# izhengfan/se2lam

Measured on NVIDIA H100. Metric: ORB keypoints/sec at 640x480 (8-level pyramid, 1000 kps/frame), higher is better.
Workload: dtype u8

## Files before the change

### se2lam_b200/csrc/orb.cu

```cuda
#include <cuda.h>

#include <algorithm>
#include <cmath>
#include <cstring>
#include <type_traits>
#include <vector>

#include "blur_px.h"
#include "common.h"
#include "fast_screen.h"
#include "introselect.h"
#include "resp_key.h"

namespace {

using se2gpu::fail;

constexpr int EDGE = 16;
constexpr int HALF_PATCH = 15;
constexpr int PATCH = 31;
constexpr int MAX_LEVELS = 16;
constexpr int FAST_THREADS = 256;
constexpr int ORB_LANES = 4;
constexpr int BLUR_WARPS = 4;
constexpr int BLUR_TH = 48;

__device__ const signed char d_pattern[1024] = {
#include "orb_pattern_31.inc"
};
__constant__ int c_umax[16];
__constant__ int c_vmax[16];
__constant__ float c_gauss[7];

struct LevelGeo {
    int w, h, pitch;
    size_t plane_off;
    int nDesired, cols, rows, nCells, nfeaturesCell;
    int cell_base;
    int kp_off, kp_cap;
    float scale, kp_size;
    int tab_off;
    int tile_base;
    int blur_th, blur_strips;
    int fbw, fbh;
    int sel_off, sel_cap;
};

struct CellGeo {
    int level, x0, y0, x1, y1;
    int skipped;
    int cand_off, cand_cap;
};

struct TileGeo { int level, strip, cg; };

struct CellHdr { int n_base, n_a, n_b, pad; };

struct OrbDev {
    int nlevels, nfeatures, fast_th, t_lo;
    int n_cells, n_tiles;
    const LevelGeo* levels;
    const CellGeo* cells;
    const TileGeo* tiles;
    const int* itab;
    const short* stab;
    uint8_t* plain;
    uint8_t* blurred;
    size_t frame_plane_bytes;
    uint32_t* cand;
    size_t cand_total;
    CellHdr* hdr;
    uint32_t* lkp;
    int lkp_total;
    int* lcount;
    uint64_t* sel;
    int sel_total;
    int* err;
    int frame0;
};

__device__ __forceinline__ int reflect101(int p, int len) {
    if (len == 1) return 0;
    while (p < 0 || p >= len) p = p < 0 ? -p : 2 * (len - 1) - p;
    return p;
}

constexpr int PYR0_ROWS = 4;
__global__ void __launch_bounds__(256) orb_pyr0(OrbDev d, LevelGeo L, const uint8_t* __restrict__ imgs, int stride, size_t frame_stride, int nvec) {
    const int tid = threadIdx.y * 64 + threadIdx.x;
    const int f = blockIdx.z + d.frame0;
    const uint8_t* img = imgs + f * frame_stride;
    uint8_t* plane = d.plain + f * d.frame_plane_bytes + L.plane_off;
    const int rows = L.h + 2 * EDGE;
    if (blockIdx.x + 1 < gridDim.x) {
        const int vx = blockIdx.x * 64 + threadIdx.x;
        const int y0 = (blockIdx.y * 4 + threadIdx.y) * PYR0_ROWS;
        if (vx >= nvec) return;
        uint4 v[PYR0_ROWS];
#pragma unroll
        for (int k = 0; k < PYR0_ROWS; ++k)
            if (y0 + k < rows) v[k] = __ldg(reinterpret_cast<const uint4*>(img + (size_t)reflect101(y0 + k - EDGE, L.h) * stride) + vx);
#pragma unroll
        for (int k = 0; k < PYR0_ROWS; ++k)
            if (y0 + k < rows) *reinterpret_cast<uint4*>(plane + (size_t)(y0 + k) * L.pitch + EDGE + 16 * vx) = v[k];
        return;
    }
    const int tail0 = EDGE + 16 * nvec, nw = 4 + (L.pitch - tail0) / 4;
    for (int item = tid; item < 4 * PYR0_ROWS * nw; item += 256) {
// ... 590 lines not shown
            if (nToRetain[k] & SEL_NOMORE) continue;
            const int t = nTotal[k];
            if (t > nNew) nToRetain[k] = nNew;
            else { nToRetain[k] = t | SEL_NOMORE; dist += nNew - t; ++more; }
        }
        nToDistribute = warp_sum(dist); nNoMore += warp_sum(more);
    }
    int before = 0, all = 0;
    for (int k = lane; k < nCells; k += 32) {
        const int kept = min(nTotal[k], nToRetain[k] & ~SEL_NOMORE);
        all += kept;
        if (k < me) before += kept;
    }
    before = warp_sum(before); all = warp_sum(all);
    __syncwarp();
    const int cap = L.sel_cap;
    if (me == 0 && lane == 0) {
        if (all > cap) *d.err = 2;
        d.lcount[f * d.nlevels + level] = min(all, cap);
    }
    const int tot = nTotal[me], n = nToRetain[me] & ~SEL_NOMORE, kept = min(tot, n);
    if (kept <= 0 || before >= cap) return;
    R* g;
    if constexpr (HARRIS) g = hb.cand64 + (size_t)f * d.cand_total + c.cand_off;
    else g = d.cand + (size_t)f * d.cand_total + c.cand_off;
    R* v = g;
    if (tot > n) {
        if (tot <= stage_n) {
            v = stage;
            for (int i = lane; i < tot; i += 32) v[i] = g[i];
            __syncwarp();
        }
        se2gpu::kp_nth_element_warp<K>(v, tot, n - 1, wq[wid]);
    }
    R* out = reinterpret_cast<R*>(d.sel) + (size_t)f * d.sel_total + L.sel_off + before;
    for (int i = lane; i < kept && before + i < cap; i += 32) out[i] = v[i];
}

template <bool HARRIS>
__global__ void __launch_bounds__(32) orb_select_levels(OrbDev d, HarrisBufs hb) {
    typedef typename std::conditional<HARRIS, se2gpu::KpKey64, se2gpu::KpScore32>::type K;
    typedef typename K::rec R;
    extern __shared__ __align__(16) uint8_t sell_smem[];
    __shared__ int wq[128];
    asm volatile("griddepcontrol.launch_dependents;" ::: "memory");
    const int lane = threadIdx.x, level = blockIdx.x, f = blockIdx.y + d.frame0;
    const LevelGeo& L = d.levels[level];
    R* v = reinterpret_cast<R*>(sell_smem);
    const R* g = reinterpret_cast<const R*>(d.sel) + (size_t)f * d.sel_total + L.sel_off;
    int* lc = d.lcount + f * d.nlevels + level;
    asm volatile("griddepcontrol.wait;" ::: "memory");
    int total = *lc;
    for (int i = lane; i < total; i += 32) v[i] = g[i];
    __syncwarp();
    if (total > L.nDesired) {
        se2gpu::kp_nth_element_warp<K>(v, total, L.nDesired - 1, wq);
        total = L.nDesired;
    }
    uint32_t* out = d.lkp + (size_t)f * d.lkp_total + L.kp_off;
    if constexpr (HARRIS) {
        float* resp = hb.lresp + (size_t)f * d.lkp_total + L.kp_off;
        for (int i = lane; i < total; i += 32) { const R r = v[i]; out[i] = (uint32_t)r; resp[i] = se2gpu::resp_from_key((uint32_t)(r >> 32)); }
    } else {
        for (int i = lane; i < total; i += 32) out[i] = v[i];
    }
    __syncwarp();
    if (lane == 0) *lc = total;
}

__global__ void __launch_bounds__(128) orb_debug_nth(uint32_t* v, const int* __restrict__ offs, const int* __restrict__ nth, int count) {
    __shared__ int wq[4][128];
    const int k = blockIdx.x * 4 + (threadIdx.x >> 5);
    if (k >= count) return;
    se2gpu::kp_nth_element_warp(v + offs[k], offs[k + 1] - offs[k], nth[k], wq[threadIdx.x >> 5]);
}

__global__ void __launch_bounds__(128) orb_debug_nth64(uint64_t* v, const int* __restrict__ offs, const int* __restrict__ nth, int count) {
    __shared__ int wq[4][128];
    const int k = blockIdx.x * 4 + (threadIdx.x >> 5);
    if (k >= count) return;
    se2gpu::kp_nth_element_warp<se2gpu::KpKey64>(v + offs[k], offs[k + 1] - offs[k], nth[k], wq[threadIdx.x >> 5]);
}

__global__ void __launch_bounds__(BLUR_WARPS * 32, 4) orb_blur(OrbDev d, int tile0, int tile_end) {
    const int tile = tile0 + blockIdx.x * BLUR_WARPS + (threadIdx.x >> 5);
    if (tile >= tile_end) return;
    const TileGeo t = d.tiles[tile];
    const LevelGeo& L = d.levels[t.level];
    const int pitch = L.pitch, Lw = L.w, Lh = L.h, th = L.blur_th, strips = L.blur_strips, ncg = pitch / 8;
    int s = t.strip, cg = t.cg + (threadIdx.x & 31);
    while (cg >= ncg) { cg -= ncg; ++s; }
    if (s >= strips) return;
    const int x8 = 8 * cg;
    const size_t off = (size_t)(blockIdx.y + d.frame0) * d.frame_plane_bytes + L.plane_off + x8;
    const uint8_t* __restrict__ src = d.plain + off;
    uint8_t* __restrict__ dst = d.blurred + off;
    if (s == 0)
        for (int y = 0; y < EDGE; ++y) *reinterpret_cast<uint2*>(dst + (size_t)y * pitch) = __ldg(reinterpret_cast<const uint2*>(src + (size_t)y * pitch));
    if (s == strips - 1)
        for (int y = EDGE + Lh; y < Lh + 2 * EDGE; ++y) *reinterpret_cast<uint2*>(dst + (size_t)y * pitch) = __ldg(reinterpret_cast<const uint2*>(src + (size_t)y * pitch));
    uint32_t m0 = 0, m1 = 0;
#pragma unroll
    for (int q = 0; q < 4; ++q) {
        m0 |= (x8 + q >= EDGE && x8 + q < EDGE + Lw) ? (0xFFu << (8 * q)) : 0u;
        m1 |= (x8 + 4 + q >= EDGE && x8 + 4 + q < EDGE + Lw) ? (0xFFu << (8 * q)) : 0u;
    }
    const int y0 = EDGE + min(s * th, Lh - th);
    const uint8_t* rp = src + (size_t)(y0 - 3) * pitch;
    uint8_t* wp = dst + (size_t)y0 * pitch;
    float hr[7][8];
    uint2 cw[7];
    uint2 nc = __ldg(reinterpret_cast<const uint2*>(rp));
    uint32_t nl = __ldg(reinterpret_cast<const uint32_t*>(rp - 4)), nr = __ldg(reinterpret_cast<const uint32_t*>(rp + 8));
    auto row = [&](const int k) {
        const uint2 c = nc;
        const uint32_t l = nl, r = nr;
        rp += pitch;
        nc = __ldg(reinterpret_cast<const uint2*>(rp));
        nl = __ldg(reinterpret_cast<const uint32_t*>(rp - 4));
        nr = __ldg(reinterpret_cast<const uint32_t*>(rp + 8));
        float b[14];
#pragma unroll
        for (int j = 0; j < 3; ++j) b[j] = blurpx::byte_to_float(l, j + 1);
#pragma unroll
        for (int j = 0; j < 4; ++j) { b[3 + j] = blurpx::byte_to_float(c.x, j); b[7 + j] = blurpx::byte_to_float(c.y, j); }
#pragma unroll
        for (int j = 0; j < 3; ++j) b[11 + j] = blurpx::byte_to_float(r, j);
#pragma unroll
        for (int q = 0; q < 8; ++q) {
            float a = __fmul_rn(c_gauss[0], b[q]);
            a = __fmaf_rn(c_gauss[1], b[q + 1], a); a = __fmaf_rn(c_gauss[2], b[q + 2], a); a = __fmaf_rn(c_gauss[3], b[q + 3], a);
            a = __fmaf_rn(c_gauss[4], b[q + 4], a); a = __fmaf_rn(c_gauss[5], b[q + 5], a); a = __fmaf_rn(c_gauss[6], b[q + 6], a);
            hr[k][q] = a;
        }
        cw[k] = c;
    };
    auto out = [&](const int k) {
        unsigned o[8];
#pragma unroll
        for (int q = 0; q < 8; ++q) {
            float a = __fmul_rn(c_gauss[3], hr[(k + 4) % 7][q]);
            a = __fmaf_rn(c_gauss[4], __fadd_rn(hr[(k + 5) % 7][q], hr[(k + 3) % 7][q]), a);
            a = __fmaf_rn(c_gauss[5], __fadd_rn(hr[(k + 6) % 7][q], hr[(k + 2) % 7][q]), a);
            a = __fmaf_rn(c_gauss[6], __fadd_rn(hr[k][q], hr[(k + 1) % 7][q]), a);
            o[q] = blurpx::round_sat_bits(a);
        }
        const uint2 ctr = cw[(k + 4) % 7];
        const uint32_t v0 = blurpx::pack_low_bytes(o[0], o[1], o[2], o[3]), v1 = blurpx::pack_low_bytes(o[4], o[5], o[6], o[7]);
        *reinterpret_cast<uint2*>(wp) = make_uint2((v0 & m0) | (ctr.x & ~m0), (v1 & m1) | (ctr.y & ~m1));
        wp += pitch;
    };
#pragma unroll
    for (int k = 0; k < 7; ++k) row(k);
    out(6);
    for (int i = 1; i < th; i += 7) {
#pragma unroll
        for (int k = 0; k < 7; ++k) { row(k); out(k); }
    }
}

__device__ __forceinline__ float fast_atan2_deg(float y, float x) {
    const float p1 = 0.9997878412794807f * (float)(180 / M_PI);
    const float p3 = -0.3258083974640975f * (float)(180 / M_PI);
    const float p5 = 0.1555786518463281f * (float)(180 / M_PI);
    const float p7 = -0.04432655554792128f * (float)(180 / M_PI);
    const float ax = fabsf(x), ay = fabsf(y);
    float a, c, c2;
    if (ax >= ay) {
        c = __fdiv_rn(ay, __fadd_rn(ax, (float)2.2204460492503131e-16));
        c2 = __fmul_rn(c, c);
        a = __fmul_rn(__fadd_rn(__fmul_rn(__fadd_rn(__fmul_rn(__fadd_rn(__fmul_rn(p7, c2), p5), c2), p3), c2), p1), c);
    } else {
        c = __fdiv_rn(ax, __fadd_rn(ay, (float)2.2204460492503131e-16));
        c2 = __fmul_rn(c, c);
        a = __fsub_rn(90.f, __fmul_rn(__fadd_rn(__fmul_rn(__fadd_rn(__fmul_rn(__fadd_rn(__fmul_rn(p7, c2), p5), c2), p3), c2), p1), c));
    }
    if (x < 0) a = __fsub_rn(180.f, a);
    if (y < 0) a = __fsub_rn(360.f, a);
    return a;
}

template <bool HARRIS>
__global__ void __launch_bounds__(256) orb_orient_describe(OrbDev d, se2gpu_keypoint* __restrict__ kps, uint8_t* __restrict__ desc,
                                                           int* __restrict__ counts, const float* __restrict__ lresp) {
    __shared__ float4 patf[256];
    for (int i = threadIdx.x; i < 256; i += blockDim.x) patf[(i & 7) * 32 + (i >> 3)] = make_float4((float)d_pattern[4 * i], (float)d_pattern[4 * i + 1], (float)d_pattern[4 * i + 2], (float)d_pattern[4 * i + 3]);
    __syncthreads();
    asm volatile("griddepcontrol.wait;" ::: "memory");
    const int f = blockIdx.y + d.frame0;
    const int slot = blockIdx.x * (blockDim.x >> 5) + (threadIdx.x >> 5);
    const int lane = threadIdx.x & 31;
    const int* lc = d.lcount + f * d.nlevels;
    int level = -1, off = 0, total = 0;
    for (int l = 0; l < d.nlevels; ++l) {
        const int c = lc[l];
        if (level < 0 && slot < total + c) { level = l; off = total; }
        total += c;
    }
    if (slot == 0 && lane == 0) counts[f] = total;
    if (level < 0) return;
    const LevelGeo& L = d.levels[level];
    const size_t kslot = (size_t)f * d.lkp_total + L.kp_off + (slot - off);
    const uint32_t rec = d.lkp[kslot];
    const int x = rec & 0xFFF, y = (rec >> 12) & 0xFFF, score = rec >> 24;
    const size_t base = f * d.frame_plane_bytes + L.plane_off + (size_t)(EDGE + y) * L.pitch + (EDGE + x);
    const uint8_t* center = d.plain + base;
    int m10 = 0, m01 = 0;
    if (lane < 31) {
        const int u = lane - HALF_PATCH, vm = c_vmax[abs(u)];
        const uint8_t* col = center + u;
        const int pitch = L.pitch;
        int colsum = col[0];
#pragma unroll
        for (int v0 = 1; v0 <= HALF_PATCH; v0 += 5) {
            int p[5], m[5];
#pragma unroll
            for (int k = 0; k < 5; ++k) {
                const int off = min(v0 + k, vm) * pitch;
                p[k] = col[off]; m[k] = col[-off];
            }
#pragma unroll
            for (int k = 0; k < 5; ++k)
                if (v0 + k <= vm) { colsum += p[k] + m[k]; m01 += (v0 + k) * (p[k] - m[k]); }
        }
        m10 = u * colsum;
    }
#pragma unroll
    for (int o = 16; o > 0; o >>= 1) { m10 += __shfl_xor_sync(0xffffffffu, m10, o); m01 += __shfl_xor_sync(0xffffffffu, m01, o); }
    const float angle = fast_atan2_deg((float)m01, (float)m10);
    const float factorPI = (float)(M_PI / 180.f);
    const float ang = __fmul_rn(angle, factorPI);
    double sd, cd;
    sincos((double)ang, &sd, &cd);
    const float a = (float)cd, b = (float)sd;
    const uint8_t* bc = d.blurred + base;
    unsigned val = 0;
    int o0[8], o1[8];
#pragma unroll
    for (int k = 0; k < 8; ++k) {
        const float4 pt = patf[k * 32 + lane];
        const float x0 = pt.x, y0 = pt.y, x1 = pt.z, y1 = pt.w;
        const int r0 = __float2int_rn(__fadd_rn(__fmul_rn(x0, b), __fmul_rn(y0, a)));
        const int c0 = __float2int_rn(__fsub_rn(__fmul_rn(x0, a), __fmul_rn(y0, b)));
        const int r1 = __float2int_rn(__fadd_rn(__fmul_rn(x1, b), __fmul_rn(y1, a)));
        const int c1 = __float2int_rn(__fsub_rn(__fmul_rn(x1, a), __fmul_rn(y1, b)));
        o0[k] = r0 * L.pitch + c0; o1[k] = r1 * L.pitch + c1;
    }
    int t0[8], t1[8];
#pragma unroll
    for (int k = 0; k < 8; ++k) { t0[k] = bc[o0[k]]; t1[k] = bc[o1[k]]; }
#pragma unroll
    for (int k = 0; k < 8; ++k) val |= (unsigned)(t0[k] < t1[k]) << k;
    unsigned w = val;
    w |= __shfl_down_sync(0xffffffffu, val, 1) << 8;
    w |= __shfl_down_sync(0xffffffffu, val, 2) << 16;
    w |= __shfl_down_sync(0xffffffffu, val, 3) << 24;
    const size_t oslot = (size_t)f * d.nfeatures + slot;
    if ((lane & 3) == 0) reinterpret_cast<unsigned*>(desc + oslot * 32)[lane >> 2] = w;
    if (lane == 0) {
        se2gpu_keypoint kp;
        kp.x = level ? __fmul_rn((float)x, L.scale) : (float)x;
        kp.y = level ? __fmul_rn((float)y, L.scale) : (float)y;
        kp.size = L.kp_size; kp.angle = angle; kp.response = HARRIS ? lresp[kslot] : (float)score; kp.octave = level; kp.class_id = -1;
        kps[oslot] = kp;
    }
}

inline int cv_round_f(float v) { return (int)lrintf(v); }

}

struct se2gpu_orb {
    int device = 0, nfeatures = 0, nlevels = 0, fast_th = 20, max_w = 0, max_h = 0, max_batch = 0;
    bool harris = false;
    double scaleFactor = 1.2;
    std::vector<float> mvScaleFactor, mvInvScaleFactor;
    std::vector<int> mnFeaturesPerLevel;
    int cur_w = -1, cur_h = -1;
    std::vector<LevelGeo> levels;
    std::vector<CellGeo> cells;
    std::vector<TileGeo> tiles;
    size_t fast_smem = 0, select_smem = 0, select_levels_smem = 0, resize_w_smem = 0;
    int sel_max_cells = 0;
    int sel_stage_n = 0;
    int resize_rows = 0, resize_raw_pitch = 0;
    int resize_tall_rows = 0; size_t resize_tall_smem = 0;
    int resize_tall_ctas = 0;
    bool fast_big = false;
    bool fast_tma = false;
    size_t fast_tma_smem = 0;
    FastMaps fast_maps{};
    bool und_on = false;
    float und_K[9] = {}, und_D[14] = {};
    int und_nd = 0, und_w = 0, und_h = 0;
    short2* d_und_m1 = nullptr; uint16_t* d_und_m2 = nullptr; size_t und_cap = 0;
    size_t cap_plane = 0, cap_cand = 0, cap_cells = 0, cap_tiles = 0, cap_tab = 0, cap_lkp = 0, cap_sel = 0;
    OrbDev d{};
    LevelGeo* d_levels = nullptr; CellGeo* d_cells = nullptr; TileGeo* d_tiles = nullptr; int* d_itab = nullptr; short* d_stab = nullptr;

    uint8_t* d_in = nullptr; se2gpu_keypoint* d_kps = nullptr; uint8_t* d_desc = nullptr; int* d_counts = nullptr;
    HarrisBufs hb{};
    se2gpu::DeviceBuffers bufs;
    int last_n = 0;
    se2gpu::Profiler prof;
    cudaStream_t side = nullptr;
    cudaEvent_t ev_pyr = nullptr, ev_blur = nullptr;
    cudaStream_t pipe[ORB_LANES] = {};
    int* pin_counts = nullptr; se2gpu_keypoint* pin_kps = nullptr; uint8_t* pin_desc = nullptr;
    struct Pending { bool on = false; int n = 0, lanes = 0; bool pipelined = false; se2gpu_keypoint* kps = nullptr; uint8_t* desc = nullptr; int* counts = nullptr;
                     se2gpu_keypoint* out_kps = nullptr; uint8_t* out_desc = nullptr; int* out_counts = nullptr; } pend;
    se2gpu_orb* twin = nullptr;
    int submit_next = 0, wait_next = 0, in_flight = 0;
    int create_args[9] = {};
};

namespace {

int build_geometry(se2gpu_orb* h, int w, int hgt, bool dry, size_t* plane_bytes, size_t* cand_total, size_t* n_cells,
                   size_t* n_tiles, size_t* tab_total, size_t* max_fast_smem,
                   std::vector<LevelGeo>* Lv, std::vector<CellGeo>* Cv, std::vector<TileGeo>* Tv, bool* fast_big_out = nullptr,
                   size_t* fast_tma_smem_out = nullptr) {
    (void)dry;
    const int nl = h->nlevels;
    std::vector<LevelGeo> L(nl);
    std::vector<CellGeo> C;
    std::vector<TileGeo> T;
    size_t poff = 0, coff = 0, toff = 0, fsm = 0, fsm_big = 0, fsm_tma = 0;
    bool fast_big = false;
    bool tma_ok = true;
    int kp_off = 0, sel_off = 0;
    const float imageRatio = (float)w / (float)hgt;
    for (int l = 0; l < nl; ++l) {
        LevelGeo& g = L[l];
        const float scale = h->mvInvScaleFactor[l];
        g.w = cv_round_f((float)w * scale); g.h = cv_round_f((float)hgt * scale);
        if (g.w < 2 * EDGE + 7 || g.h < 2 * EDGE + 7) return fail(SE2GPU_ERR_INVALID, "level %d of a %dx%d frame is %dx%d: too small for the 16 px border", l, w, hgt, g.w, g.h);
        if (g.w + 2 * EDGE > 4095 || g.h + 2 * EDGE > 4095) return fail(SE2GPU_ERR_CAPACITY, "frames wider/taller than 4063 px are not supported");
        g.pitch = (g.w + 2 * EDGE + 31) & ~31;
        g.plane_off = poff;
        poff += (size_t)g.pitch * (g.h + 2 * EDGE);
        poff = (poff + 255) & ~(size_t)255;
        g.nDesired = h->mnFeaturesPerLevel[l];
        g.cols = (int)sqrtf((float)g.nDesired / (5 * imageRatio));
        g.rows = (int)(imageRatio * g.cols);
        if (g.cols < 1 || g.rows < 1) return fail(SE2GPU_ERR_INVALID, "level %d has a %dx%d cell grid (nfeatures too small): undefined in the reference", l, g.cols, g.rows);
        const int minB = EDGE, maxBX = g.w - EDGE, maxBY = g.h - EDGE;
        const int W = maxBX - minB, H = maxBY - minB;
        const int cellW = (int)ceilf((float)W / g.cols), cellH = (int)ceilf((float)H / g.rows);
        g.nCells = g.rows * g.cols;
        g.nfeaturesCell = (int)ceilf((float)g.nDesired / g.nCells);
        g.cell_base = (int)C.size();
        g.kp_off = kp_off; g.kp_cap = g.nDesired; kp_off += g.nDesired;
        g.scale = h->mvScaleFactor[l];
        g.kp_size = (float)(int)(PATCH * h->mvScaleFactor[l]);
        g.tab_off = (int)toff; toff += (size_t)g.w + g.h;
        std::vector<int> iniXCol(g.cols, 0);
        const size_t first_cell = C.size();
        int max_cw = 0, max_ch = 0;
        float hY = cellH + 6;
        for (int i = 0; i < g.rows; ++i) {
            const float iniY = minB + i * cellH - 3;
            bool rowSkipped = false;
            if (i == g.rows - 1) { hY = maxBY + 3 - iniY; if (hY <= 0) rowSkipped = true; }
            float hX = cellW + 6;
            for (int j = 0; j < g.cols; ++j) {
                CellGeo c{};
                c.level = l;
                if (rowSkipped) { c.skipped = 1; C.push_back(c); continue; }
                float iniX;
                if (i == 0) { iniX = minB + j * cellW - 3; iniXCol[j] = (int)iniX; } else iniX = iniXCol[j];
                if (j == g.cols - 1) { hX = maxBX + 3 - iniX; if (hX <= 0) { c.skipped = 1; C.push_back(c); continue; } }
                const int r0 = (int)iniY, r1 = (int)(iniY + hY), c0 = (int)iniX, c1 = (int)(iniX + hX);
                if (r1 > g.h || c1 > g.w || r0 < 0 || c0 < 0) return fail(SE2GPU_ERR_INVALID, "cell grid of level %d leaves the image (the reference asserts here)", l);
                c.x0 = c0 + 3; c.x1 = c1 - 3; c.y0 = r0 + 3; c.y1 = r1 - 3;
                const int cw = std::max(c.x1 - c.x0, 0), chh = std::max(c.y1 - c.y0, 0);
                c.cand_off = (int)coff;
                c.cand_cap = ((cw + 1) / 2) * ((chh + 1) / 2) + 8;
                coff += c.cand_cap;
                if (cw > 0 && chh > 0) {
                    max_cw = std::max(max_cw, ((c.x0 - 3 + EDGE) & 15) + cw); max_ch = std::max(max_ch, chh);
                    const size_t pwb = (size_t)((cw + 6 + 3 + 3) / 4 + 1) * 4;
                    const size_t bitmap = (size_t)chh * fastpx::nms_words_per_row(cw) * 4;
                    if (pwb * (chh + 6) > 65535) fast_big = true;
                    fsm = std::max(fsm, ((pwb * (chh + 6) + 15) & ~(size_t)15) + (((size_t)fastpx::nms_plane_bytes((int)pwb, chh) + 15) & ~(size_t)15) + bitmap + (size_t)cw * chh * 2 + 64);
                    const size_t nchunk = (size_t)chh * ((cw + 31) / 32);
                    fsm_big = std::max(fsm_big, ((pwb * (chh + 6) + 15) & ~(size_t)15) + (((size_t)(cw + 2) * (chh + 2) + 15) & ~(size_t)15) + nchunk * 4 + 64);
                }
                C.push_back(c);
            }
        }
        g.fbw = (max_cw + 6 + 15) & ~15; g.fbh = max_ch + 6;
        if (max_cw > 0) {
            if (g.fbw > 256 || g.fbh > 256 || (size_t)g.fbw * g.fbh > 65535) tma_ok = false;
            for (size_t ci = first_cell; ci < C.size(); ++ci) {
                const int cw = C[ci].x1 - C[ci].x0, chh = C[ci].y1 - C[ci].y0;
                if (C[ci].skipped || cw <= 0 || chh <= 0) continue;
                const size_t pw = (size_t)g.fbw, bitmap = (size_t)chh * fastpx::nms_words_per_row(cw) * 4;
                fsm_tma = std::max(fsm_tma, (size_t)128 + ((pw * g.fbh + 15) & ~(size_t)15) + (((size_t)fastpx::nms_plane_bytes(g.fbw, chh) + 15) & ~(size_t)15) + bitmap + (size_t)cw * chh * 2 + 64);
            }
        }
        g.sel_cap = 2 * g.nDesired + 4 * g.nCells + 64;
        g.sel_off = sel_off; sel_off += g.sel_cap;
        g.tile_base = (int)T.size();
        g.blur_strips = std::max(2, (g.h + BLUR_TH - 1) / BLUR_TH);
        g.blur_th = ((g.h + g.blur_strips - 1) / g.blur_strips + 12) / 7 * 7 - 6;
        for (int it = 0; it < g.blur_strips * (g.pitch / 8); it += 32) T.push_back(TileGeo{l, it / (g.pitch / 8), it % (g.pitch / 8)});
    }
    *plane_bytes = poff; *cand_total = coff; *n_cells = C.size(); *n_tiles = T.size(); *tab_total = toff;
    if (fsm > 227 * 1024) fast_big = true;
    *max_fast_smem = fast_big ? fsm_big : fsm;
    if (fast_big_out) *fast_big_out = fast_big;
    if (fast_tma_smem_out) *fast_tma_smem_out = (tma_ok && !fast_big && fsm_tma <= 227 * 1024) ? fsm_tma : 0;
    if (Lv) *Lv = L;
    if (Cv) *Cv = C;
    if (Tv) *Tv = T;
    return SE2GPU_OK;
}

typedef CUresult (*EncodeTiledFn)(CUtensorMap*, CUtensorMapDataType, cuuint32_t, void*, const cuuint64_t*, const cuuint64_t*, const cuuint32_t*,
                                  const cuuint32_t*, CUtensorMapInterleave, CUtensorMapSwizzle, CUtensorMapL2promotion, CUtensorMapFloatOOBfill);
EncodeTiledFn tensor_map_encoder() {
    static EncodeTiledFn fn = [] {
        void* p = nullptr;
        cudaDriverEntryPointQueryResult q = cudaDriverEntryPointSymbolNotFound;
        if (cudaGetDriverEntryPoint("cuTensorMapEncodeTiled", &p, cudaEnableDefault, &q) != cudaSuccess || q != cudaDriverEntryPointSuccess) { cudaGetLastError(); p = nullptr; }
        return (EncodeTiledFn)p;
    }();
    return fn;
}

constexpr int BLUR_SPLIT = 1;
constexpr int PIPE_CHUNKS = 4, PIPE_FIRST_PCT = 50, SUBMIT_CHUNKS = 1;

bool encode_fast_maps(se2gpu_orb* h, size_t frame_plane_bytes) {
    EncodeTiledFn enc = tensor_map_encoder();
    if (!enc || (frame_plane_bytes & 15)) return false;
    for (int l = 0; l < h->nlevels; ++l) {
        const LevelGeo& g = h->levels[l];
        if (g.fbw <= 6) { memset(&h->fast_maps.m[l], 0, sizeof(CUtensorMap)); continue; }
        const cuuint64_t gdim[3] = {(cuuint64_t)g.pitch, (cuuint64_t)(g.h + 2 * EDGE), (cuuint64_t)h->max_batch};
        const cuuint64_t gstr[2] = {(cuuint64_t)g.pitch, (cuuint64_t)frame_plane_bytes};
        const cuuint32_t box[3] = {(cuuint32_t)g.fbw, (cuuint32_t)g.fbh, 1u};
        const cuuint32_t estr[3] = {1u, 1u, 1u};
        void* base = h->d.plain + g.plane_off;
        if (((uintptr_t)base & 15) || (g.pitch & 15)) return false;
        if (enc(&h->fast_maps.m[l], CU_TENSOR_MAP_DATA_TYPE_UINT8, 3, base, gdim, gstr, box, estr, CU_TENSOR_MAP_INTERLEAVE_NONE,
                CU_TENSOR_MAP_SWIZZLE_NONE, CU_TENSOR_MAP_L2_PROMOTION_L2_128B, CU_TENSOR_MAP_FLOAT_OOB_FILL_NONE) != CUDA_SUCCESS) return false;
    }
    return true;
}

int set_geometry(se2gpu_orb* h, int w, int hgt, cudaStream_t s) {
    if (w == h->cur_w && hgt == h->cur_h) return SE2GPU_OK;
    size_t pb, ct, nc, nt, tt, fsm, fsm_tma = 0;
    bool big = false;
    int rc = build_geometry(h, w, hgt, false, &pb, &ct, &nc, &nt, &tt, &fsm, &h->levels, &h->cells, &h->tiles, &big, &fsm_tma);
    if (rc != SE2GPU_OK) return rc;
    if (pb > h->cap_plane || ct > h->cap_cand || nc > h->cap_cells || nt > h->cap_tiles || tt > h->cap_tab)
        return fail(SE2GPU_ERR_CAPACITY, "frame %dx%d exceeds the capacity this extractor was created with (%dx%d)", w, hgt, h->max_w, h->max_h);
    if (fsm > 227 * 1024) return fail(SE2GPU_ERR_CAPACITY, "a FAST cell of a %dx%d frame needs %zu B of shared memory", w, hgt, fsm);
    std::vector<int> itab(tt, 0);
    std::vector<short> stab(2 * tt, 0);
    for (int l = 1; l < h->nlevels; ++l) {
        const LevelGeo& g = h->levels[l];
        const LevelGeo& sg = h->levels[l - 1];
        const double scale_x = 1. / ((double)g.w / sg.w), scale_y = 1. / ((double)g.h / sg.h);
        int* xofs = itab.data() + g.tab_off; int* yofs = xofs + g.w;
        short* ialpha = stab.data() + 2 * (size_t)g.tab_off; short* ibeta = ialpha + 2 * g.w;
        for (int dx = 0; dx < g.w; ++dx) {
            float fx = (float)((dx + 0.5) * scale_x - 0.5);
            int sx = (int)floorf(fx);
            fx -= sx;
            if (sx < 0) { fx = 0; sx = 0; }
            if (sx >= sg.w - 1) { fx = 0; sx = sg.w - 1; }
            xofs[dx] = sx;
            ialpha[2 * dx] = (short)std::min(std::max(cv_round_f((1.f - fx) * 2048.f), -32768), 32767);
            ialpha[2 * dx + 1] = (short)std::min(std::max(cv_round_f(fx * 2048.f), -32768), 32767);
        }
        for (int dy = 0; dy < g.h; ++dy) {
            float fy = (float)((dy + 0.5) * scale_y - 0.5);
            int sy = (int)floorf(fy);
            fy -= sy;
            yofs[dy] = sy;
            ibeta[2 * dy] = (short)cv_round_f((1.f - fy) * 2048.f);
            ibeta[2 * dy + 1] = (short)cv_round_f(fy * 2048.f);
        }
    }
    SE2_CUDA(cudaMemcpyAsync(h->d_levels, h->levels.data(), sizeof(LevelGeo) * h->levels.size(), cudaMemcpyHostToDevice, s));
    SE2_CUDA(cudaMemcpyAsync(h->d_cells, h->cells.data(), sizeof(CellGeo) * h->cells.size(), cudaMemcpyHostToDevice, s));
    SE2_CUDA(cudaMemcpyAsync(h->d_tiles, h->tiles.data(), sizeof(TileGeo) * h->tiles.size(), cudaMemcpyHostToDevice, s));
    SE2_CUDA(cudaMemcpyAsync(h->d_itab, itab.data(), sizeof(int) * itab.size(), cudaMemcpyHostToDevice, s));
    SE2_CUDA(cudaMemcpyAsync(h->d_stab, stab.data(), sizeof(short) * stab.size(), cudaMemcpyHostToDevice, s));
    SE2_CUDA(cudaStreamSynchronize(s));
    h->fast_smem = fsm; h->fast_big = big;
    {
        double ratio = 1.0;
        for (size_t l = 1; l < h->levels.size(); ++l)
            ratio = std::max(ratio, std::max((double)h->levels[l - 1].w / h->levels[l].w, (double)h->levels[l - 1].h / h->levels[l].h));
        h->resize_rows = (int)ceil(RESIZE_TR * ratio) + 4;
        h->resize_raw_pitch = (((int)ceil(128 * ratio) + 4 + 15 + 15) / 16) * 16;
        h->resize_w_smem = (size_t)h->resize_rows * (128 * sizeof(uint16_t) + h->resize_raw_pitch) + 16;
        if (h->resize_w_smem > 200 * 1024) return fail(SE2GPU_ERR_CAPACITY, "scale factor %.3f needs %zu B of shared memory in orb_resize_w", ratio, h->resize_w_smem);
        SE2_CUDA(cudaFuncSetAttribute(orb_resize_w<RESIZE_TR>, cudaFuncAttributeMaxDynamicSharedMemorySize, (int)h->resize_w_smem));
        h->resize_tall_rows = (int)ceil(RESIZE_TR_TALL * ratio) + 4;
        h->resize_tall_smem = (size_t)h->resize_tall_rows * (128 * sizeof(uint16_t) + h->resize_raw_pitch) + 16;
        h->resize_tall_ctas = 0;
        if (h->resize_tall_smem <= 200 * 1024) {
            SE2_CUDA(cudaFuncSetAttribute(orb_resize_w<RESIZE_TR_TALL>, cudaFuncAttributeMaxDynamicSharedMemorySize, (int)h->resize_tall_smem));
            int per_sm = 0, sms = 0;
            SE2_CUDA(cudaOccupancyMaxActiveBlocksPerMultiprocessor(&per_sm, orb_resize_w<RESIZE_TR_TALL>, 256, h->resize_tall_smem));
            SE2_CUDA(cudaDeviceGetAttribute(&sms, cudaDevAttrMultiProcessorCount, h->device));
            h->resize_tall_ctas = per_sm * sms;
        }
    }
    SE2_CUDA(cudaFuncSetAttribute(orb_fast_cells_big, cudaFuncAttributeMaxDynamicSharedMemorySize, (int)std::max<size_t>(fsm, 1024)));
    SE2_CUDA(cudaFuncSetAttribute(orb_fast_cells<false>, cudaFuncAttributeMaxDynamicSharedMemorySize, (int)std::max<size_t>(fsm, 1024)));
    h->fast_tma = fsm_tma > 0 && encode_fast_maps(h, pb);
    h->fast_tma_smem = fsm_tma;
    if (h->fast_tma) SE2_CUDA(cudaFuncSetAttribute(orb_fast_cells<true>, cudaFuncAttributeMaxDynamicSharedMemorySize, (int)std::max<size_t>(fsm_tma, 1024)));
    int max_cells = 0, sel_total = 0, max_sel_cap = 0, max_cand = 0;
    for (const LevelGeo& g : h->levels) { max_cells = std::max(max_cells, g.nCells); max_sel_cap = std::max(max_sel_cap, g.sel_cap); sel_total += g.sel_cap; }
    for (const CellGeo& c : h->cells) max_cand = std::max(max_cand, c.skipped ? 0 : c.cand_cap);
    const int rec = h->harris ? 8 : 4;
    const int stage_n = std::min((max_cand + 31) & ~31, SEL_STAGE_BYTES / rec);
    const size_t ssm = (size_t)SEL_WARPS * ((size_t)stage_n * rec + 2 * 4 * (size_t)max_cells);
    if ((size_t)sel_total > h->cap_sel) return fail(SE2GPU_ERR_CAPACITY, "frame %dx%d exceeds the selection capacity this extractor was created with", w, hgt);
    const size_t lsm = (size_t)max_sel_cap * (h->harris ? 8 : 4);
    if (ssm > 227 * 1024 || lsm > 227 * 1024) return fail(SE2GPU_ERR_CAPACITY, "the selection of a %dx%d frame needs %zu / %zu B of shared memory", w, hgt, ssm, lsm);
    if (h->harris) {
        SE2_CUDA(cudaFuncSetAttribute(orb_select_cells<true>, cudaFuncAttributeMaxDynamicSharedMemorySize, (int)ssm));
        SE2_CUDA(cudaFuncSetAttribute(orb_select_levels<true>, cudaFuncAttributeMaxDynamicSharedMemorySize, (int)lsm));
    } else {
        SE2_CUDA(cudaFuncSetAttribute(orb_select_cells<false>, cudaFuncAttributeMaxDynamicSharedMemorySize, (int)ssm));
        SE2_CUDA(cudaFuncSetAttribute(orb_select_levels<false>, cudaFuncAttributeMaxDynamicSharedMemorySize, (int)lsm));
    }
    h->select_smem = ssm; h->select_levels_smem = lsm; h->sel_max_cells = max_cells; h->sel_stage_n = stage_n;
// ... 56 lines not shown
    }
    return SE2GPU_OK;
}

int ensure_undistort_map(se2gpu_orb* h, int w, int hgt, cudaStream_t s) {
    if (h->und_w == w && h->und_h == hgt) return SE2GPU_OK;
    std::vector<short2> m1; std::vector<uint16_t> m2;
    int rc = build_undistort_map(h->und_K, h->und_D, h->und_nd, w, hgt, m1, m2);
    if (rc != SE2GPU_OK) return rc;
    const size_t px = (size_t)w * hgt;
    if (px > h->und_cap) {
        if (h->d_und_m1) cudaFree(h->d_und_m1);
        if (h->d_und_m2) cudaFree(h->d_und_m2);
        h->d_und_m1 = nullptr; h->d_und_m2 = nullptr; h->und_cap = 0;
        SE2_CUDA(cudaMalloc((void**)&h->d_und_m1, px * sizeof(short2)));
        SE2_CUDA(cudaMalloc((void**)&h->d_und_m2, px * sizeof(uint16_t)));
        h->und_cap = px;
    }
    SE2_CUDA(cudaMemcpyAsync(h->d_und_m1, m1.data(), px * sizeof(short2), cudaMemcpyHostToDevice, s));
    SE2_CUDA(cudaMemcpyAsync(h->d_und_m2, m2.data(), px * sizeof(uint16_t), cudaMemcpyHostToDevice, s));
    SE2_CUDA(cudaStreamSynchronize(s));
    h->und_w = w; h->und_h = hgt;
    return SE2GPU_OK;
}

template <typename... KArgs, typename... Args>
cudaError_t launch_pdl(void (*kernel)(KArgs...), dim3 grid, dim3 block, size_t smem, cudaStream_t s, Args... args) {
    cudaLaunchConfig_t cfg = {};
    cfg.gridDim = grid; cfg.blockDim = block; cfg.dynamicSmemBytes = smem; cfg.stream = s;
    cudaLaunchAttribute at[1];
    at[0].id = cudaLaunchAttributeProgrammaticStreamSerialization;
    at[0].val.programmaticStreamSerializationAllowed = 1;
    cfg.attrs = at; cfg.numAttrs = 1;
    ::se2gpu::g_launches.fetch_add(1, std::memory_order_relaxed);
    return cudaLaunchKernelEx(&cfg, kernel, args...);
}

int run_device(se2gpu_orb* h, const uint8_t* d_imgs, int n, int w, int hgt, int stride, size_t frame_stride,
               se2gpu_keypoint* d_kps, uint8_t* d_desc, int* d_counts, cudaStream_t s, int frame0 = 0, int lane = -1) {
    int rc = set_geometry(h, w, hgt, s);
    if (rc != SE2GPU_OK) return rc;
    if (h->und_on && (rc = ensure_undistort_map(h, w, hgt, s)) != SE2GPU_OK) return rc;
    OrbDev d = h->d;
    d.frame0 = frame0;
    cudaStream_t side = lane < 0 ? h->side : nullptr;
    cudaEvent_t ev_pyr = h->ev_pyr, ev_blur = h->ev_blur;
    se2gpu::Profiler& pr = h->prof;
    SE2_NVTX("se2gpu.orb.run_device");
    nvtxRangePushA("se2gpu.orb.pyramid");
    pr.begin(0, s);
    {
        const LevelGeo& g = h->levels[0];
        if (h->und_on) {
            dim3 grid((g.pitch / 4 + 127) / 128, g.h + 2 * EDGE, n);
            SE2_LAUNCH(orb_pyr0_undistort, grid, 128, 0, s, d, g, d_imgs, stride, frame_stride, h->d_und_m1, h->d_und_m2);
        } else {
            const int aligned = (((uintptr_t)d_imgs | (uintptr_t)stride | (uintptr_t)frame_stride) & 15) == 0;
            const int nvec = aligned ? g.w / 16 : 0;
            dim3 grid((nvec + 63) / 64 + 1, (g.h + 2 * EDGE + 4 * PYR0_ROWS - 1) / (4 * PYR0_ROWS), n);
            SE2_LAUNCH(orb_pyr0, grid, dim3(64, 4), 0, s, d, g, d_imgs, stride, frame_stride, nvec);
        }
    }
    const bool overlap = !pr.on && side != nullptr;
    for (int l = 1; l < h->nlevels; ++l) {
        const LevelGeo& g = h->levels[l];
        cudaLaunchConfig_t cfg = {};
        const int ncx = (g.pitch + 127) / 128, H = g.h + 2 * EDGE;
        const int tall_grid = ncx * ((H + RESIZE_TR_TALL - 1) / RESIZE_TR_TALL) * n;
        const bool tall = h->resize_tall_ctas > 0 && tall_grid >= h->resize_tall_ctas;
        const int tr = tall ? RESIZE_TR_TALL : RESIZE_TR;
        cfg.gridDim = dim3(ncx, (H + tr - 1) / tr, n);
        cfg.blockDim = dim3(32, 8); cfg.dynamicSmemBytes = tall ? h->resize_tall_smem : h->resize_w_smem; cfg.stream = s;
        cudaLaunchAttribute at[1];
        at[0].id = cudaLaunchAttributeProgrammaticStreamSerialization;
        at[0].val.programmaticStreamSerializationAllowed = 1;
        cfg.attrs = at; cfg.numAttrs = 1;
        if (tall) SE2_CUDA(cudaLaunchKernelEx(&cfg, orb_resize_w<RESIZE_TR_TALL>, d, g, h->levels[l - 1], h->resize_tall_rows, h->resize_raw_pitch));
        else SE2_CUDA(cudaLaunchKernelEx(&cfg, orb_resize_w<RESIZE_TR>, d, g, h->levels[l - 1], h->resize_rows, h->resize_raw_pitch));
        ::se2gpu::g_launches.fetch_add(1, std::memory_order_relaxed);
    }
    if (overlap) SE2_CUDA(cudaEventRecord(ev_pyr, s));
    pr.end(s);
    nvtxRangePop();
    auto launch_blur = [&](cudaStream_t st, int t0, int t1) {
        if (t1 > t0) SE2_LAUNCH(orb_blur, dim3((t1 - t0 + BLUR_WARPS - 1) / BLUR_WARPS, n), BLUR_WARPS * 32, 0, st, d, t0, t1);
    };
    const int split = std::min(BLUR_SPLIT, h->nlevels);
    const int tilesA = split < h->nlevels ? h->levels[split].tile_base : d.n_tiles;
    if (overlap) {
        SE2_CUDA(cudaStreamWaitEvent(side, ev_pyr, 0));
        launch_blur(side, 0, tilesA);
        launch_blur(side, tilesA, d.n_tiles);
        SE2_CUDA(cudaEventRecord(ev_blur, side));
    }
    SE2_NVTX("se2gpu.orb.fast_select_blur_describe");
    pr.begin(1, s);
    if (h->fast_big) SE2_LAUNCH(orb_fast_cells_big, dim3(d.n_cells, n), FAST_THREADS, h->fast_smem, s, d);
    else if (h->fast_tma) SE2_CUDA(launch_pdl(orb_fast_cells<true>, dim3(d.n_cells, n), FAST_THREADS, h->fast_tma_smem, s, d, h->fast_maps));
    else SE2_CUDA(launch_pdl(orb_fast_cells<false>, dim3(d.n_cells, n), FAST_THREADS, h->fast_smem, s, d, h->fast_maps));
    if (h->harris) SE2_LAUNCH(orb_harris, dim3(d.n_cells, n), HARRIS_THREADS, 0, s, d, h->hb.cand64);
    pr.end(s);
    pr.begin(2, s);
    const dim3 sel_grid(n, (d.n_cells + SEL_WARPS - 1) / SEL_WARPS);
    if (h->harris) {
        SE2_CUDA(launch_pdl(orb_select_cells<true>, sel_grid, SEL_WARPS * 32, h->select_smem, s, d, h->hb, h->sel_max_cells, h->sel_stage_n));
        SE2_CUDA(launch_pdl(orb_select_levels<true>, dim3(h->nlevels, n), 32, h->select_levels_smem, s, d, h->hb));
    } else {
        SE2_CUDA(launch_pdl(orb_select_cells<false>, sel_grid, SEL_WARPS * 32, h->select_smem, s, d, h->hb, h->sel_max_cells, h->sel_stage_n));
        SE2_CUDA(launch_pdl(orb_select_levels<false>, dim3(h->nlevels, n), 32, h->select_levels_smem, s, d, h->hb));
    }
    pr.end(s);
    if (overlap) {
        SE2_CUDA(cudaStreamWaitEvent(s, ev_blur, 0));
    } else {
        pr.begin(3, s);
        launch_blur(s, 0, d.n_tiles);
        pr.end(s);
    }
    const int warps = 8;
    const dim3 desc_grid((h->nfeatures + warps - 1) / warps, n);
    pr.begin(4, s);
    if (h->harris) SE2_CUDA(launch_pdl(orb_orient_describe<true>, desc_grid, warps * 32, 0, s, d, d_kps, d_desc, d_counts, (const float*)h->hb.lresp));
    else SE2_CUDA(launch_pdl(orb_orient_describe<false>, desc_grid, warps * 32, 0, s, d, d_kps, d_desc, d_counts, (const float*)h->hb.lresp));
    pr.end(s);
    h->last_n = std::max(h->last_n * (frame0 > 0), frame0 + n);
    return SE2GPU_OK;
}

}

int se2gpu::orb_prepare_shape(se2gpu_orb* h, int w, int hgt, cudaStream_t s) {
    SE2_CUDA(cudaSetDevice(h->device));
    int rc = set_geometry(h, w, hgt, s);
    if (rc == SE2GPU_OK && h->und_on) rc = ensure_undistort_map(h, w, hgt, s);
    return rc;
}

extern "C" {

se2gpu_orb* se2gpu_orb_create_scored(int nfeatures, float scale_factor, int nlevels, int score_type, int fast_th, int max_w, int max_h,
                                     int max_batch, int device) {
    if (score_type != SE2GPU_ORB_HARRIS_SCORE && score_type != SE2GPU_ORB_FAST_SCORE) {
        fail(SE2GPU_ERR_INVALID, "unknown ORB score type %d (HARRIS_SCORE = 0, FAST_SCORE = 1)", score_type); return nullptr;
    }
    if (nfeatures <= 0 || nlevels <= 0 || nlevels > MAX_LEVELS || !(scale_factor > 1.0f) || fast_th < 1 || fast_th > 254 ||
        max_w <= 0 || max_h <= 0 || max_batch <= 0) { fail(SE2GPU_ERR_INVALID, "bad ORB parameters"); return nullptr; }
    if (se2gpu::select_device(device) != SE2GPU_OK) return nullptr;
    se2gpu_orb* h = new se2gpu_orb;
    h->device = device; h->nfeatures = nfeatures; h->nlevels = nlevels; h->fast_th = fast_th;
    h->harris = score_type == SE2GPU_ORB_HARRIS_SCORE;
    h->max_w = max_w; h->max_h = max_h; h->max_batch = max_batch;
    { int* a = h->create_args; a[0] = nfeatures; memcpy(&a[1], &scale_factor, sizeof(float)); a[2] = nlevels; a[3] = fast_th; a[4] = max_w; a[5] = max_h; a[6] = max_batch; a[7] = device; a[8] = score_type; }
    h->scaleFactor = scale_factor;
    h->mvScaleFactor.resize(nlevels); h->mvInvScaleFactor.resize(nlevels); h->mnFeaturesPerLevel.resize(nlevels);
    h->mvScaleFactor[0] = 1;
    for (int i = 1; i < nlevels; i++) h->mvScaleFactor[i] = (float)(h->mvScaleFactor[i - 1] * h->scaleFactor);
    const float invScaleFactor = (float)(1.0f / h->scaleFactor);
    h->mvInvScaleFactor[0] = 1;
    for (int i = 1; i < nlevels; i++) h->mvInvScaleFactor[i] = h->mvInvScaleFactor[i - 1] * invScaleFactor;
    const float factor = (float)(1.0 / h->scaleFactor);
    float nDesired = nfeatures * (1 - factor) / (1 - (float)pow((double)factor, (double)nlevels));
    int sum = 0;
    for (int l = 0; l < nlevels - 1; l++) { h->mnFeaturesPerLevel[l] = cv_round_f(nDesired); sum += h->mnFeaturesPerLevel[l]; nDesired *= factor; }
    h->mnFeaturesPerLevel[nlevels - 1] = std::max(nfeatures - sum, 0);
    if (sum > nfeatures) { fail(SE2GPU_ERR_INVALID, "per-level quotas sum to %d > nfeatures %d for these parameters", sum, nfeatures); delete h; return nullptr; }
    int umax[16];
    {
        int v, v0, vmax = (int)floorf(HALF_PATCH * sqrtf(2.f) / 2 + 1), vmin = (int)ceilf(HALF_PATCH * sqrtf(2.f) / 2);
        const double hp2 = HALF_PATCH * HALF_PATCH;
        for (v = 0; v <= vmax; ++v) umax[v] = (int)lrint(sqrt(hp2 - v * v));
        for (v = HALF_PATCH, v0 = 0; v >= vmin; --v) { while (umax[v0] == umax[v0 + 1]) ++v0; umax[v] = v0; ++v0; }
    }
    float gk[7];
    { double g[7], s = 0; for (int i = 0; i < 7; ++i) { double x = i - 3; g[i] = std::exp(-0.5 * x * x / 4.0); s += g[i]; } for (int i = 0; i < 7; ++i) gk[i] = (float)(g[i] * (1. / s)); }
    size_t pb, ct, nc, nt, tt, fsm;
    int rc = build_geometry(h, max_w, max_h, true, &pb, &ct, &nc, &nt, &tt, &fsm, nullptr, nullptr, nullptr);
    if (rc != SE2GPU_OK) { delete h; return nullptr; }
    h->cap_plane = pb + 4096; h->cap_cand = ct + ct / 8 + 4096; h->cap_cells = nc + 64; h->cap_tiles = nt + 64; h->cap_tab = tt + 64;
    h->cap_lkp = nfeatures + 64;
    h->cap_sel = 2 * (size_t)nfeatures + 4 * h->cap_cells + 64 * (size_t)nlevels;
    const size_t B = max_batch;
    bool ok = true;
    auto A = [&](auto** p, size_t c) { ok = ok && h->bufs.alloc(p, c) == cudaSuccess; };
    OrbDev& d = h->d;
    A(&h->d_levels, (size_t)nlevels); A(&h->d_cells, h->cap_cells); A(&h->d_tiles, h->cap_tiles); A(&h->d_itab, h->cap_tab); A(&h->d_stab, 2 * h->cap_tab);
    A(&d.plain, B * h->cap_plane); A(&d.blurred, B * h->cap_plane);
    A(&d.cand, B * h->cap_cand); A(&d.hdr, B * h->cap_cells); A(&d.lkp, B * h->cap_lkp); A(&d.lcount, B * nlevels); A(&d.sel, B * h->cap_sel); A(&d.err, 1);
    A(&h->d_in, B * (size_t)max_w * max_h); A(&h->d_kps, B * nfeatures); A(&h->d_desc, B * nfeatures * 32); A(&h->d_counts, B);
    if (h->harris) { A(&h->hb.cand64, B * h->cap_cand); A(&h->hb.lresp, B * h->cap_lkp); }
    if (!ok) { fail(SE2GPU_ERR_CUDA, "device allocation failed (%s)", cudaGetErrorString(cudaGetLastError())); se2gpu_orb_destroy(h); return nullptr; }
    cudaMemset(d.err, 0, sizeof(int));
    if (cudaStreamCreateWithFlags(&h->side, cudaStreamNonBlocking) != cudaSuccess || cudaEventCreateWithFlags(&h->ev_pyr, cudaEventDisableTiming) != cudaSuccess ||
        cudaEventCreateWithFlags(&h->ev_blur, cudaEventDisableTiming) != cudaSuccess) { h->side = nullptr; cudaGetLastError(); }
    for (int l = 0; l < ORB_LANES && h->side; ++l)
        if (cudaStreamCreateWithFlags(&h->pipe[l], cudaStreamNonBlocking) != cudaSuccess) { h->pipe[l] = nullptr; cudaGetLastError(); break; }
    cudaMemcpyToSymbol(c_umax, umax, sizeof umax);
    {
        int vmax[16];
        for (int u = 0; u <= HALF_PATCH; ++u) { vmax[u] = 0; for (int v = 0; v <= HALF_PATCH; ++v) if (umax[v] >= u) vmax[u] = v; }
// ... 250 lines not shown
```

Baseline: 113.6 million.

## Auto-tune blur strip height via makespan model and chain blur launches with PDL

```diff
diff --git a/se2lam_b200/csrc/orb.cu b/se2lam_b200/csrc/orb.cu
--- a/se2lam_b200/csrc/orb.cu
+++ b/se2lam_b200/csrc/orb.cu
@@ -3,6 +3,7 @@
 #include <algorithm>
 #include <cmath>
 #include <cstring>
+#include <queue>
 #include <type_traits>
 #include <vector>
 
@@ -23,7 +24,8 @@
 constexpr int FAST_THREADS = 256;
 constexpr int ORB_LANES = 4;
 constexpr int BLUR_WARPS = 4;
-constexpr int BLUR_TH = 48;
+constexpr int BLUR_TH_MIN = 22, BLUR_TH_MAX = 64;
+constexpr int BLUR_SPLIT = 1;
 
 __device__ const signed char d_pattern[1024] = {
 #include "orb_pattern_31.inc"
@@ -780,7 +782,7 @@
     se2gpu::kp_nth_element_warp<se2gpu::KpKey64>(v + offs[k], offs[k + 1] - offs[k], nth[k], wq[threadIdx.x >> 5]);
 }
 
-__global__ void __launch_bounds__(BLUR_WARPS * 32, 4) orb_blur(OrbDev d, int tile0, int tile_end) {
+__device__ __forceinline__ void blur_strip(const OrbDev& d, int tile0, int tile_end) {
     const int tile = tile0 + blockIdx.x * BLUR_WARPS + (threadIdx.x >> 5);
     if (tile >= tile_end) return;
     const TileGeo t = d.tiles[tile];
@@ -857,6 +859,12 @@
     }
 }
 
+__global__ void __launch_bounds__(BLUR_WARPS * 32, 5) orb_blur(OrbDev d, int tile0, int tile_end) {
+    asm volatile("griddepcontrol.launch_dependents;" ::: "memory");
+    blur_strip(d, tile0, tile_end);
+    asm volatile("griddepcontrol.wait;" ::: "memory");
+}
+
 __device__ __forceinline__ float fast_atan2_deg(float y, float x) {
     const float p1 = 0.9997878412794807f * (float)(180 / M_PI);
     const float p3 = -0.3258083974640975f * (float)(180 / M_PI);
@@ -984,6 +992,7 @@
     int resize_rows = 0, resize_raw_pitch = 0;
     int resize_tall_rows = 0; size_t resize_tall_smem = 0;
     int resize_tall_ctas = 0;
+    int blur_ctas = 0;
     bool fast_big = false;
     bool fast_tma = false;
     size_t fast_tma_smem = 0;
@@ -1014,11 +1023,60 @@
 
 namespace {
 
+int blur_strips_for(const LevelGeo& g, int target, int* th) {
+    const int strips = std::max(2, (g.h + target - 1) / target);
+    *th = ((g.h + strips - 1) / strips + 12) / 7 * 7 - 6;
+    return strips;
+}
+
+long blur_makespan(const std::vector<LevelGeo>& L, int a, int b, const int* target, int frames, int slots) {
+    std::vector<int> cost;
+    int in_cta = 0;
+    for (int l = a; l < b; ++l) {
+        int th;
+        const int items = blur_strips_for(L[l], target[l], &th) * (L[l].pitch / 8);
+        for (int it = 0; it < items; it += 32) {
+            if (in_cta++ % BLUR_WARPS == 0) cost.push_back(0);
+            cost.back() = std::max(cost.back(), th + 6);
+        }
+    }
+    std::priority_queue<long, std::vector<long>, std::greater<long>> free_at;
+    for (int k = 0; k < slots; ++k) free_at.push(0);
+    long end = 0;
+    for (int f = 0; f < frames; ++f)
+        for (int c : cost) {
+            const long t = free_at.top() + c;
+            free_at.pop(); free_at.push(t); end = std::max(end, t);
+        }
+    return end;
+}
+
+void blur_split(const se2gpu_orb* h, std::vector<LevelGeo>& L, bool dry, std::vector<TileGeo>* T) {
+    const int nl = (int)L.size();
+    int target[MAX_LEVELS];
+    for (int a = 0, b; a < nl; a = b) {
+        b = a < BLUR_SPLIT ? std::min(BLUR_SPLIT, nl) : nl;
+        int best = BLUR_TH_MIN;
+        long best_end = -1;
+        for (int t = BLUR_TH_MIN; !dry && h->blur_ctas > 0 && t <= BLUR_TH_MAX; t += 7) {
+            for (int l = a; l < b; ++l) target[l] = t;
+            const long end = blur_makespan(L, a, b, target, h->max_batch, h->blur_ctas);
+            if (best_end < 0 || end < best_end) { best = t; best_end = end; }
+        }
+        for (int l = a; l < b; ++l) target[l] = best;
+    }
+    for (int l = 0; l < nl; ++l) {
+        LevelGeo& g = L[l];
+        g.tile_base = (int)T->size();
+        g.blur_strips = blur_strips_for(g, target[l], &g.blur_th);
+        for (int it = 0; it < g.blur_strips * (g.pitch / 8); it += 32) T->push_back(TileGeo{l, it / (g.pitch / 8), it % (g.pitch / 8)});
+    }
+}
+
 int build_geometry(se2gpu_orb* h, int w, int hgt, bool dry, size_t* plane_bytes, size_t* cand_total, size_t* n_cells,
                    size_t* n_tiles, size_t* tab_total, size_t* max_fast_smem,
                    std::vector<LevelGeo>* Lv, std::vector<CellGeo>* Cv, std::vector<TileGeo>* Tv, bool* fast_big_out = nullptr,
                    size_t* fast_tma_smem_out = nullptr) {
-    (void)dry;
     const int nl = h->nlevels;
     std::vector<LevelGeo> L(nl);
     std::vector<CellGeo> C;
@@ -1099,11 +1157,8 @@
         }
         g.sel_cap = 2 * g.nDesired + 4 * g.nCells + 64;
         g.sel_off = sel_off; sel_off += g.sel_cap;
-        g.tile_base = (int)T.size();
-        g.blur_strips = std::max(2, (g.h + BLUR_TH - 1) / BLUR_TH);
-        g.blur_th = ((g.h + g.blur_strips - 1) / g.blur_strips + 12) / 7 * 7 - 6;
-        for (int it = 0; it < g.blur_strips * (g.pitch / 8); it += 32) T.push_back(TileGeo{l, it / (g.pitch / 8), it % (g.pitch / 8)});
-    }
+    }
+    blur_split(h, L, dry, &T);
     *plane_bytes = poff; *cand_total = coff; *n_cells = C.size(); *n_tiles = T.size(); *tab_total = toff;
     if (fsm > 227 * 1024) fast_big = true;
     *max_fast_smem = fast_big ? fsm_big : fsm;
@@ -1127,7 +1182,6 @@
     return fn;
 }
 
-constexpr int BLUR_SPLIT = 1;
 constexpr int PIPE_CHUNKS = 4, PIPE_FIRST_PCT = 50, SUBMIT_CHUNKS = 1;
 
 bool encode_fast_maps(se2gpu_orb* h, size_t frame_plane_bytes) {
@@ -1150,6 +1204,12 @@
 
 int set_geometry(se2gpu_orb* h, int w, int hgt, cudaStream_t s) {
     if (w == h->cur_w && hgt == h->cur_h) return SE2GPU_OK;
+    if (h->blur_ctas == 0) {
+        int per_sm = 0, sms = 0;
+        SE2_CUDA(cudaOccupancyMaxActiveBlocksPerMultiprocessor(&per_sm, orb_blur, BLUR_WARPS * 32, 0));
+        SE2_CUDA(cudaDeviceGetAttribute(&sms, cudaDevAttrMultiProcessorCount, h->device));
+        h->blur_ctas = per_sm * sms;
+    }
     size_t pb, ct, nc, nt, tt, fsm, fsm_tma = 0;
     bool big = false;
     int rc = build_geometry(h, w, hgt, false, &pb, &ct, &nc, &nt, &tt, &fsm, &h->levels, &h->cells, &h->tiles, &big, &fsm_tma);
@@ -1372,15 +1432,19 @@
     if (overlap) SE2_CUDA(cudaEventRecord(ev_pyr, s));
     pr.end(s);
     nvtxRangePop();
-    auto launch_blur = [&](cudaStream_t st, int t0, int t1) {
-        if (t1 > t0) SE2_LAUNCH(orb_blur, dim3((t1 - t0 + BLUR_WARPS - 1) / BLUR_WARPS, n), BLUR_WARPS * 32, 0, st, d, t0, t1);
+    auto launch_blur = [&](cudaStream_t st, int t0, int t1, bool pdl) {
+        if (t1 <= t0) return cudaSuccess;
+        const dim3 grid((t1 - t0 + BLUR_WARPS - 1) / BLUR_WARPS, n);
+        if (pdl) return launch_pdl(orb_blur, grid, BLUR_WARPS * 32, 0, st, d, t0, t1);
+        SE2_LAUNCH(orb_blur, grid, BLUR_WARPS * 32, 0, st, d, t0, t1);
+        return cudaSuccess;
     };
     const int split = std::min(BLUR_SPLIT, h->nlevels);
     const int tilesA = split < h->nlevels ? h->levels[split].tile_base : d.n_tiles;
     if (overlap) {
         SE2_CUDA(cudaStreamWaitEvent(side, ev_pyr, 0));
-        launch_blur(side, 0, tilesA);
-        launch_blur(side, tilesA, d.n_tiles);
+        SE2_CUDA(launch_blur(side, 0, tilesA, false));
+        SE2_CUDA(launch_blur(side, tilesA, d.n_tiles, tilesA > 0));
         SE2_CUDA(cudaEventRecord(ev_blur, side));
     }
     SE2_NVTX("se2gpu.orb.fast_select_blur_describe");
@@ -1404,7 +1468,7 @@
         SE2_CUDA(cudaStreamWaitEvent(s, ev_blur, 0));
     } else {
         pr.begin(3, s);
-        launch_blur(s, 0, d.n_tiles);
+        SE2_CUDA(launch_blur(s, 0, d.n_tiles, false));
         pr.end(s);
     }
     const int warps = 8;
```

Result: slower. 112.1 million, median of 6 (-1.3%).
